# wamuumu/query-recommendation-system

Measured on AMD Instinct MI355X. Metric: MinHash signatures/sec through the whole hot path (signatures -> LSH candidates -> pair scoring -> top-K), higher is better.
Workload: dtype u16/int32 MinHash values, uint64 keys and pairs (integer); float64 cosine

## Files before the change

include/qrlsh.h:

```cpp
#ifndef QRLSH_H
#define QRLSH_H

#include <stddef.h>
#include <stdint.h>

#ifdef __cplusplus
extern "C" {
#endif

#define QRLSH_OK 0
#define QRLSH_EINVAL (-1)
#define QRLSH_EHIP (-2)
#define QRLSH_EUNSUPPORTED (-3)
#define QRLSH_EWORKSPACE (-4)

#define QRLSH_PERM_U16 0
#define QRLSH_PERM_I32 1

#define QRLSH_SIG_I32 0
#define QRLSH_SIG_U16 1

#define QRLSH_SORT_MIX 1u
#define QRLSH_SORT_IOTA 2u
#define QRLSH_SORT_FOLD 4u
// ... 65 lines not shown
                              void *stream);
int qrlsh_region_unique_fill(const uint64_t *tmp, int64_t n, int32_t group_bits, int64_t nids, const void *workspace,
                             uint64_t *out, void *stream);

size_t qrlsh_pair_regions_words(int64_t n, int64_t nids, int32_t group_bits, double words_per_query);
size_t qrlsh_pair_regions_tmp_words(int64_t n, int64_t nids, int32_t group_bits, double words_per_query);
int64_t qrlsh_pair_regions_cap(int64_t n, int64_t nids, int32_t group_bits, double words_per_query);
int64_t qrlsh_pair_regions_count(int64_t n, int64_t nids, int32_t group_bits, double words_per_query);
int qrlsh_pair_regions_scatter32(const uint64_t *words, int64_t n, int32_t group_bits, int32_t id_bits, int64_t nids,
                                 double words_per_query, uint64_t *tmp_regions, uint32_t *regions, uint32_t *counts,
                                 uint32_t *overflow_out, void *stream);
int qrlsh_region_unique_count_regions32(const uint32_t *regions, const uint32_t *counts, int64_t cap, int64_t n,
                                        int32_t group_bits, int32_t id_bits, int64_t nids, uint64_t *tmp, void *workspace,
                                        size_t workspace_bytes, const uint32_t *scatter_overflow, uint64_t *out3,
                                        void *stream);

int qrlsh_row_norms(const int32_t *sig, int64_t nq, int32_t P, int64_t *norm2_out, void *stream);
int qrlsh_verify_pairs(const void *sig, int32_t sig_dtype, int32_t P, int32_t b, const uint64_t *pairs,
                       int64_t n, uint8_t *flags_out, void *stream);
int qrlsh_score_pairs(const void *sig, int32_t sig_dtype, const int64_t *norm2, int32_t P,
                      const uint64_t *pairs, int64_t n, int32_t *milli_out, double *cos_out,
                      uint64_t *edge_out, int32_t id_bits, uint32_t *edge_dst_out, void *stream);

int qrlsh_topk_count(const uint64_t *sorted_edges, int64_t n_edges, int32_t K, int32_t id_bits,
                     void *workspace, size_t workspace_bytes, uint64_t *total_out, void *stream);
int qrlsh_topk_fill(const uint64_t *sorted_edges, const uint32_t *sorted_dst, int64_t n_edges, int32_t K,
                    int32_t id_bits, const void *workspace, int32_t *src_out, int32_t *dst_out,
                    int32_t *milli_out, void *stream);
int qrlsh_topk_fill_based(const uint64_t *sorted_edges, const uint32_t *sorted_dst, int64_t n_edges, int32_t K,
                          int32_t id_bits, int64_t src_base, const void *workspace, int32_t *src_out,
// ... 264 lines not shown
```

query-recommendation-system_amd/csrc/bucket.hip:

```cpp
#include "common.h"


__device__ static inline uint64_t rec_x(uint64_t word, int xbits) { return word & ((1ull << xbits) - 1ull); }
__device__ static inline uint64_t rec_word(uint64_t x, uint32_t id_hi, int xbits) {
  return rec_x(x, xbits) | (uint64_t)id_hi << xbits;
}
__device__ static inline uint32_t rec_id(uint64_t word, uint16_t tail, int xbits) {
  return (uint32_t)(word >> xbits) << 16 | tail;
}

struct PartPool {
  uint64_t *keys;
  uint16_t *vals;
  unsigned long long *cursor;
  uint32_t cap;
  uint4 *runs;
  unsigned long long *nruns;
  uint32_t runs_max;
  uint32_t *fill;
  uint32_t slot_base;
};

#ifndef QR_PS_IPT
#define QR_PS_IPT 16
// ... 790 lines not shown
QRLSH_EXPORT size_t qrlsh_bucket_part_words(int64_t nq, int32_t b, int32_t part_bits) {
  if (nq <= 0 || b <= 0) return 0;
  const size_t plain = (size_t)b * nq;
  const size_t regions = region_words(nq, b, part_bits) + pool_records(nq, b);
  return regions > plain ? regions : plain;
}
QRLSH_EXPORT size_t qrlsh_bucket_tmp_words(int64_t nq, int32_t b, int32_t part_bits) {
  if (nq <= 0 || b <= 0 || part_bits <= 8) return 0;
  const size_t plain = (size_t)b * nq;
  const int c1 = coarse_bits(part_bits);
  const int64_t slab = 1ll << slab_bits(part_bits);
  const size_t regions = (((size_t)b * n_slabs(nq, part_bits)) << c1) * coarse_region(nq < slab ? nq : slab, c1);
  return regions > plain ? regions : plain;
}

QRLSH_EXPORT int qrlsh_bucket_pairs_emit(const uint64_t *keys, uint64_t *part_keys, uint32_t *part_ids,
                                         uint64_t *tmp_keys, uint32_t *tmp_ids, int64_t nq, int32_t b, int32_t r,
                                         int32_t part_bits, void *workspace, size_t workspace_bytes,
                                         uint64_t *pairs_out, uint64_t capacity, uint64_t *total_overflow_out,
                                         void *stream) {
  return qrlsh_bucket_pairs_emit_chunked(keys, 0, 0, 0, part_keys, part_ids, tmp_keys, tmp_ids, nq, b, r, part_bits,
                                         workspace, workspace_bytes, pairs_out, capacity, total_overflow_out, stream);
}

QRLSH_EXPORT int qrlsh_bucket_pairs_emit_chunked(const uint64_t *keys, int64_t key_chunk, int64_t key_chunk_stride,
                                                 int64_t key_band_stride, uint64_t *part_keys, uint32_t *part_ids,
                                                 uint64_t *tmp_keys, uint32_t *tmp_ids, int64_t nq, int32_t b,
                                                 int32_t r, int32_t part_bits, void *workspace,
                                                 size_t workspace_bytes, uint64_t *pairs_out, uint64_t capacity,
                                                 uint64_t *total_overflow_out, void *stream) {
  QR_CHECK_ARG(key_chunk >= 0 && key_chunk_stride >= 0 && key_band_stride >= 0,
               "qrlsh_bucket_pairs_emit_chunked: bad key layout");
  hipStream_t st = static_cast<hipStream_t>(stream);
  const int rc = bucket_check("qrlsh_bucket_pairs_emit", keys, part_keys, part_ids, tmp_keys, tmp_ids, nq, b, r,
                              part_bits, workspace, workspace_bytes, total_overflow_out, st);
  if (rc != QRLSH_OK || nq == 0) return rc;
  QR_CHECK_ARG(pairs_out || capacity == 0, "qrlsh_bucket_pairs_emit: null output with capacity %llu",
               (unsigned long long)capacity);
  uint32_t *ovf = reinterpret_cast<uint32_t *>(total_overflow_out + 1);
  if (nq > (1ll << (16 + part_bits))) {
    if (hipMemsetAsync(ovf, 1, 1, st) != hipSuccess) {
      qrlsh_set_error("qrlsh_bucket_pairs_emit: hipMemsetAsync failed");
      return QRLSH_EHIP;
    }
    return QRLSH_OK;
  }
  const int nparts = 1 << part_bits;
  const BucketWs w = bucket_ws(workspace, nq, b, part_bits);
// ... 16 lines not shown
  pool.cap = (uint32_t)pool_records(nq, b);
  pool.runs = w.runs;
  pool.runs_max = POOL_RUNS;
  pool.fill = w.fill;
  pool.slot_base = 0;
  PartPool no_pool = pool;
  no_pool.keys = nullptr;
  no_pool.vals = nullptr;
  constexpr int MAX_GROUPS = EMIT_MAX_GROUPS;
  unsigned long long *nbig0 = w.nbig;
  uint64_t *biglist0 = w.biglist;
  const uint64_t slots = (uint64_t)b << T;
  const bool small_parts = two && small_form(nq, T);
  const int ntiles = (int)ceil_div64(nq, PS_TILE);
  const int64_t band_words = key_band_stride ? key_band_stride : nq;
  const int GROUPS = (int64_t)b * nq >= (64ll << 20) ? MAX_GROUPS : 1;
  const int per = (b + GROUPS - 1) / GROUPS;
  const int ngroups = (b + per - 1) / per;
  const uint64_t list_room = (slots - MAX_GROUPS) / (uint64_t)ngroups;
  const uint32_t big_max = (uint32_t)(list_room < FIN_BIG_LIST ? list_room : FIN_BIG_LIST);
  if (hipMemsetAsync(cur1, 0, (((size_t)b * nslabs) << c1) * sizeof(uint32_t), st) != hipSuccess ||
      (two && hipMemsetAsync(cur2, 0, ((size_t)b << T) * sizeof(uint32_t), st) != hipSuccess) ||
      hipMemsetAsync(w.fill, 0xFF, ((size_t)b << T) * sizeof(uint32_t), st) != hipSuccess ||
      hipMemsetAsync(w.poolctl, 0, 16, st) != hipSuccess ||
      hipMemsetAsync(nbig0, 0, MAX_GROUPS * sizeof(unsigned long long), st) != hipSuccess ||
      (ngroups > 1 && hipMemsetAsync(w.runs, 0, (size_t)POOL_RUNS * sizeof(uint4), st) != hipSuccess)) {
    qrlsh_set_error("qrlsh_bucket_pairs_emit: hipMemsetAsync failed");
    return QRLSH_EHIP;
  }
  hipStream_t aux = nullptr;
  int gi = 0;
  for (int g0 = 0; g0 < b; g0 += per, ++gi) {
    const int nb = (b - g0 < per) ? b - g0 : per;
    hipStream_t s = (aux && (gi & 1)) ? aux : st;
    uint64_t *biglist = biglist0 + (size_t)gi * big_max;
    unsigned long long *nbig = nbig0 + gi;
    uint64_t *k1 = two ? tmp_keys : part_keys;
    uint16_t *v1 = two ? tmp_tails : part_tails;
    pool.slot_base = (uint32_t)((size_t)g0 << T);
    BigDesc *desc = w.desc + (size_t)gi * FIN_BIG_LIST;
    const size_t in0 = ((size_t)g0 * nslabs) << c1;
    QR_PART_SCATTER(false, dim3(ntiles, nb), dim3(SORT_THREADS), 0, s, keys + (size_t)g0 * band_words,
                    (const uint16_t *)nullptr, k1 + in0 * cap1, v1 + in0 * cap1, nq, ntiles, 64 - c1, (1u << c1) - 1u,
                    cur1 + in0, cap1, ovf, qr_empty_key(r), (const uint32_t *)nullptr, 0u, key_chunk, key_chunk_stride,
                    key_band_stride, c1, nslabs, slab_shift, two ? no_pool : pool);
    if (two)
      QR_PART_SCATTER(true, dim3((unsigned)ceil_div64(cap1, PS_TILE), (nb * nslabs) << c1), dim3(SORT_THREADS), 0, s,
                      (const uint64_t *)tmp_keys + in0 * cap1, (const uint16_t *)tmp_tails + in0 * cap1,
                      part_keys + ((size_t)g0 << T) * cap2, part_tails + ((size_t)g0 << T) * cap2, (int64_t)0, 0, 64 - T,
                      lowmask, cur2 + ((size_t)g0 << T), cap2, ovf, qr_empty_key(r), (const uint32_t *)cur1 + in0, cap1,
                      (int64_t)0, (int64_t)0, (int64_t)0, c1, nslabs, slab_shift, pool);
    if (gi == 0 && b > per) aux = qr_aux_fork(st);
    const uint32_t slot0 = (uint32_t)((size_t)g0 << T);
    const uint64_t *gkeys = part_keys + (size_t)slot0 * cap2;
    const uint16_t *gids = part_tails + (size_t)slot0 * cap2;
    const uint32_t *gcounts = cur2 + slot0;
    if (small_parts && T >= 12)
      QR_LAUNCH("bucket_emit", bucket_finish_packed_kernel, dim3(nparts, nb), dim3(FIN_PK_THREADS), 0, s, gkeys, gids, nparts,
                64 - T, total_overflow_out, ovf, pairs_out, capacity, gcounts, cap2, biglist, nbig, big_max, slot0);
    else if (small_parts)
      QR_LAUNCH("bucket_emit", (bucket_finish_kernel<FIN_SMALL_THREADS, FIN_SMALL_CAP>), dim3(nparts, nb),
                dim3(FIN_SMALL_THREADS), 0, s, gkeys, gids, nparts, 64 - T, total_overflow_out, ovf, pairs_out, capacity, gcounts,
                cap2, biglist, nbig, big_max, slot0);
    else
      QR_LAUNCH("bucket_emit", (bucket_finish_kernel<>), dim3(nparts, nb), dim3(FIN_THREADS), 0, s, gkeys, gids, nparts, 64 - T,
                total_overflow_out, ovf, pairs_out, capacity, gcounts, cap2, biglist, nbig, big_max, slot0);
    QR_LAUNCH("bucket_emit_big", bucket_big_gather_kernel, dim3(64), dim3(256), 0, s, (const uint64_t *)biglist,
              (const unsigned long long *)nbig, big_max, desc, (const uint64_t *)part_keys, (const uint16_t *)part_tails,
              (const uint32_t *)cur2, cap2, pool, g_big_limit, ovf);
    QR_LAUNCH("bucket_emit_big", bucket_finish_big_kernel, dim3(FIN_BIG_GRID), dim3(FIN_THREADS), 0, s,
              (const uint64_t *)part_keys, (const uint16_t *)part_tails, (const uint64_t *)pool.keys,
              (const uint16_t *)pool.vals, 64 - T, (const BigDesc *)desc, (const unsigned long long *)nbig, big_max,
              total_overflow_out, pairs_out, capacity);
  }
  if (aux && qr_aux_join(st) != QRLSH_OK) return QRLSH_EHIP;
  QR_LAUNCH_CHECK("qrlsh_bucket_pairs_emit");
  return QRLSH_OK;
#undef QR_PART_SCATTER
}
```

query-recommendation-system_amd/csrc/dedup.hip:

```cpp
#include "common.h"
#include <type_traits>

struct RowSplit {
  int gbits, jbits;
  __device__ uint32_t row(uint64_t x) const { return (uint32_t)(x >> (32 + gbits)); }
  __device__ uint32_t val(uint64_t x) const {
    const uint32_t j = (uint32_t)x;
    return gbits ? ((uint32_t)(x >> 32) & ((1u << gbits) - 1u)) << jbits | j : j;
  }
  __device__ uint64_t word(uint64_t x0, uint32_t v) const {
    if (!gbits) return (x0 & 0xFFFFFFFF00000000ull) | v;
    const uint64_t i = ((x0 >> 32) & ~(uint64_t)((1u << gbits) - 1u)) | (v >> jbits);
    return i << 32 | (v & ((1u << jbits) - 1u));
  }
};

constexpr int RD_THREADS = 512;
constexpr int RD_C = 2048;
constexpr int RD_CAP = 1024;
constexpr int RD_IMG = RD_C + RD_CAP;
constexpr int RD_PER = RD_IMG / RD_THREADS;
constexpr uint32_t RD_EMPTY = 0xFFFFFFFFu;

__global__ __launch_bounds__(RD_THREADS) void row_unique_kernel(const uint64_t *__restrict__ in, int64_t n,
// ... 640 lines not shown
static_assert(PG_IPT_N2 % 4 == 0, "level 2 of the narrow form reads four entries per load");
static_assert(SORT_THREADS * (PG_IPT > PG_IPT_N1 ? (PG_IPT > PG_IPT_N2 ? PG_IPT : PG_IPT_N2) : (PG_IPT_N1 > PG_IPT_N2 ? PG_IPT_N1 : PG_IPT_N2)) < 0xFFFF,
              "a word's place in its tile is kept in 16 bits");
constexpr int PG_LDS_FIXED = RADIX * 9 + 16;
constexpr int pg_wgs(int ipt, int staged_bytes) {
  const int w = 160 * 1024 / (SORT_THREADS * ipt * staged_bytes + PG_LDS_FIXED);
  return w > 4 ? 4 : w < 1 ? 1 : w;
}
enum { PG_IN_WORDS = 0, PG_IN_TMP_NARROW = 2 };
enum { PG_OUT_VALUES = 1, PG_OUT_NARROW = 2 };
constexpr int pg_staged_bytes(int out) { return out == PG_OUT_VALUES ? 5 : 6; }
template <int IN, int OUT, int IPT>
__global__ __launch_bounds__(SORT_THREADS, pg_wgs(IPT, pg_staged_bytes(OUT))) void pair_group_scatter_kernel(
    const void *__restrict__ in_, const uint8_t *__restrict__ in_tails, void *__restrict__ out_, uint8_t *__restrict__ out_tails,
    int64_t n_in, int ntiles, int shift, uint32_t dmask, uint32_t *__restrict__ cursors, uint32_t cap,
    uint32_t *__restrict__ overflow, const uint32_t *__restrict__ in_counts, uint32_t in_cap, int gbits, int jbits, uint32_t bmask) {
  constexpr bool LEVEL2 = IN != PG_IN_WORDS;
  constexpr int TILE = SORT_THREADS * IPT;
  using D = typename std::conditional<OUT == PG_OUT_NARROW, uint16_t, uint8_t>::type;
  static_assert(IN == PG_IN_WORDS || IN == PG_IN_TMP_NARROW, "pair words or the tmp regions of a first level");
  static_assert(OUT == PG_OUT_NARROW ? IN == PG_IN_WORDS : OUT == PG_OUT_VALUES, "tmp regions are dealt into the final regions");
  __shared__ uint32_t cnt[RADIX];
  __shared__ uint32_t lsum[SORT_THREADS / WAVE];
  __shared__ uint32_t gdelta[RADIX];
  __shared__ uint8_t gok[RADIX];
  __shared__ __attribute__((aligned(16))) unsigned char stage[TILE * pg_staged_bytes(OUT)];
  uint32_t *const spay = reinterpret_cast<uint32_t *>(stage);
  D *const sdig = reinterpret_cast<D *>(stage + TILE * 4);
  const int tile = LEVEL2 ? (int)blockIdx.x : xcd_tile(blockIdx.x, ntiles), batch = blockIdx.y;
  const int lane = threadIdx.x & (WAVE - 1), w = threadIdx.x >> 6;
  const int64_t n = LEVEL2 ? (int64_t)min(in_counts[batch], in_cap) : n_in;
  const int64_t tbase = (int64_t)tile * TILE;
  if (tbase >= n) return;
  cnt[threadIdx.x] = 0;
  __syncthreads();
  const size_t boff = LEVEL2 ? (size_t)batch * in_cap : 0;
  const uint32_t nd = dmask + 1u;
  uint32_t pay[IPT];
  uint32_t dr[IPT];
  if constexpr (IN == PG_IN_TMP_NARROW) {
    const uint32_t *vals = static_cast<const uint32_t *>(in_) + boff;
    const uint8_t *tails = in_tails + boff;
    uint32_t tl[IPT / 4];
#pragma unroll
    for (int q = 0; q < IPT / 4; ++q) {
      const int64_t idx = tbase + ((int64_t)q * SORT_THREADS + threadIdx.x) * 4;
// ... 120 lines not shown
}
QRLSH_EXPORT size_t qrlsh_pair_regions_tmp_words(int64_t n, int64_t nids, int32_t group_bits, double words_per_query) {
  if (n <= 0 || nids <= 0 || group_bits < 0 || group_bits > 8) return 0;
  const PairRegions r = pair_regions(n, nids, group_bits, words_per_query);
  return r.ra ? (size_t)r.na * r.cap_a : 0;
}
QRLSH_EXPORT int64_t qrlsh_pair_regions_cap(int64_t n, int64_t nids, int32_t group_bits, double words_per_query) {
  if (n <= 0 || nids <= 0 || group_bits < 0 || group_bits > 8) return 0;
  return (int64_t)pair_regions(n, nids, group_bits, words_per_query).cap_b;
}
QRLSH_EXPORT int64_t qrlsh_pair_regions_count(int64_t n, int64_t nids, int32_t group_bits, double words_per_query) {
  if (n <= 0 || nids <= 0 || group_bits < 0 || group_bits > 8) return 0;
  return pair_regions(n, nids, group_bits, words_per_query).nregions;
}

QRLSH_EXPORT int qrlsh_pair_regions_scatter32(const uint64_t *words, int64_t n, int32_t group_bits, int32_t id_bits,
                                              int64_t nids, double words_per_query, uint64_t *tmp_regions, uint32_t *regions,
                                              uint32_t *counts, uint32_t *overflow_out, void *stream) {
  QR_CHECK_ARG(group_bits >= 0 && group_bits <= 8 && id_bits >= 1 && id_bits <= 31 && nids > 0 && nids <= (1ll << id_bits) &&
                   (group_bits + id_bits < 32 || (group_bits + id_bits == 32 && nids < (1ll << id_bits))),
               "qrlsh_pair_regions_scatter32: group_bits=%d / id_bits=%d / nids=%lld do not fit a 32-bit value", group_bits,
               id_bits, (long long)nids);
  QR_CHECK_ARG(n >= 0 && n < (1ll << 32) && counts && overflow_out, "qrlsh_pair_regions_scatter32: bad arguments");
  hipStream_t st = static_cast<hipStream_t>(stream);
  const PairRegions r = pair_regions(n > 0 ? n : 1, nids, group_bits, words_per_query);
  QR_CHECK_ARG(r.rbits <= 16 && r.na <= RADIX, "qrlsh_pair_regions_scatter32: %d region bits", r.rbits);
  QR_CHECK_ARG(pair_regions_fit_u32(r),
               "qrlsh_pair_regions_scatter32: regions reach 2^32 words (na * cap_a = %llu, 2^rb * cap_b = %llu; need both < 2^32)",
               (unsigned long long)r.na * r.cap_a, (unsigned long long)r.cap_b << r.rb);
  if (hipMemsetAsync(counts, 0, ((size_t)r.nregions + RADIX) * sizeof(uint32_t), st) != hipSuccess ||
      hipMemsetAsync(overflow_out, 0, sizeof(uint32_t), st) != hipSuccess) {
    qrlsh_set_error("qrlsh_pair_regions_scatter32: hipMemsetAsync failed");
    return QRLSH_EHIP;
  }
  if (n == 0) return QRLSH_OK;
  QR_CHECK_ARG(words && regions && (r.ra == 0 || tmp_regions), "qrlsh_pair_regions_scatter32: null pointer");
  const int sh = 32 + group_bits;
  const uint32_t *none = nullptr;
  if (r.ra == 0) {
    const int ntiles = (int)ceil_div64(n, SORT_THREADS * PG_IPT);
    QR_LAUNCH("pair_group", (pair_group_scatter_kernel<PG_IN_WORDS, PG_OUT_VALUES, PG_IPT>), dim3(ntiles, 1), dim3(SORT_THREADS), 0, st,
              (const void *)words, (const uint8_t *)nullptr, (void *)regions, (uint8_t *)nullptr, n, ntiles, sh,
              (1u << r.rb) - 1u, counts, r.cap_b, overflow_out, none, 0u, (int)group_bits, (int)id_bits, 0u);
  } else {
    QR_CHECK_ARG((reinterpret_cast<uintptr_t>(tmp_regions) & 15u) == 0, "qrlsh_pair_regions_scatter32: tmp_regions not 16-byte aligned");
    uint32_t *cur_a = counts + r.nregions;
    uint32_t *tvals = reinterpret_cast<uint32_t *>(tmp_regions);
    uint8_t *ttails = reinterpret_cast<uint8_t *>(tvals + (size_t)r.na * r.cap_a);
    const int ntiles = (int)ceil_div64(n, SORT_THREADS * PG_IPT_N1);
    QR_LAUNCH("pair_group", (pair_group_scatter_kernel<PG_IN_WORDS, PG_OUT_NARROW, PG_IPT_N1>), dim3(ntiles, 1), dim3(SORT_THREADS),
              0, st, (const void *)words, (const uint8_t *)nullptr, (void *)tvals, ttails, n, ntiles, sh + r.rb, (1u << r.ra) - 1u,
              cur_a, r.cap_a, overflow_out, none, 0u, (int)group_bits, (int)id_bits, (1u << r.rb) - 1u);
    QR_LAUNCH("pair_group", (pair_group_scatter_kernel<PG_IN_TMP_NARROW, PG_OUT_VALUES, PG_IPT_N2>),
              dim3((unsigned)ceil_div64(r.cap_a, SORT_THREADS * PG_IPT_N2), (unsigned)r.na), dim3(SORT_THREADS), 0, st,
              (const void *)tvals, (const uint8_t *)ttails, (void *)regions, (uint8_t *)nullptr, (int64_t)0, 0, 0, (1u << r.rb) - 1u,
              counts, r.cap_b, overflow_out, (const uint32_t *)cur_a, r.cap_a, 0, 0, 0u);
  }
  QR_LAUNCH_CHECK("qrlsh_pair_regions_scatter32");
  return QRLSH_OK;
}
```

query-recommendation-system_amd/qrlsh/_lib.py:

```python
import ctypes
import os

_HERE = os.path.dirname(os.path.abspath(__file__))
LIB_PATH = os.environ.get("QRLSH_LIB", os.path.join(_HERE, "libqrlsh.so"))

QRLSH_OK = 0
QRLSH_EINVAL = -1
QRLSH_EHIP = -2
QRLSH_EUNSUPPORTED = -3
QRLSH_EWORKSPACE = -4

PERM_U16 = 0
PERM_I32 = 1
SIG_I32 = 0
SIG_U16 = 1
SORT_MIX = 1
SORT_IOTA = 2
SORT_FOLD = 4
SORT_OWNER = 8
SORT_HOST = 16
SUM_PAIRWISE = 0
SUM_SEQUENTIAL = 1
RECOMMEND_MAX_K = 1024
INDEX_MAX_K = 256
# ... 29 lines not shown
    "qrlsh_bucket_part_words": (_sz, [_i64, _i32, _i32]),
    "qrlsh_set_big_part_limit": (_i64, [_i64]),
    "qrlsh_set_score_runs": (_i32, [_i32]),
    "qrlsh_bucket_tmp_words": (_sz, [_i64, _i32, _i32]),
    "qrlsh_bucket_pairs_emit": (ctypes.c_int, [_vp, _vp, _vp, _vp, _vp, _i64, _i32, _i32, _i32, _vp, _sz, _vp, _u64, _vp, _vp]),
    "qrlsh_compact_workspace_bytes": (_sz, [_i64]),
    "qrlsh_row_unique_workspace_bytes": (_sz, [_i64]),
    "qrlsh_row_unique_count": (ctypes.c_int, [_vp, _i64, _i32, _i32, _vp, _vp, _sz, _vp, _vp]),
    "qrlsh_row_unique_fill": (ctypes.c_int, [_vp, _i64, _vp, _vp, _vp]),
    "qrlsh_region_unique_workspace_bytes": (_sz, [_i64, _i32]),
    "qrlsh_region_unique_count": (ctypes.c_int, [_vp, _i64, _i32, _i32, _i64, _vp, _vp, _sz, _vp, _vp]),
    "qrlsh_region_unique_fill": (ctypes.c_int, [_vp, _i64, _i32, _i64, _vp, _vp, _vp]),
    "qrlsh_region_unique_count_regions32": (ctypes.c_int, [_vp, _vp, _i64, _i64, _i32, _i32, _i64, _vp, _vp, _sz, _vp, _vp,
                                                           _vp]),
    "qrlsh_pair_regions_scatter32": (ctypes.c_int, [_vp, _i64, _i32, _i32, _i64, ctypes.c_double, _vp, _vp, _vp, _vp, _vp]),
    "qrlsh_pair_regions_words": (_sz, [_i64, _i64, _i32, ctypes.c_double]),
    "qrlsh_pair_regions_tmp_words": (_sz, [_i64, _i64, _i32, ctypes.c_double]),
    "qrlsh_pair_regions_cap": (_i64, [_i64, _i64, _i32, ctypes.c_double]),
    "qrlsh_pair_regions_count": (_i64, [_i64, _i64, _i32, ctypes.c_double]),
    "qrlsh_unique_count": (ctypes.c_int, [_vp, _i64, _vp, _sz, _vp, _vp]),
    "qrlsh_unique_fill": (ctypes.c_int, [_vp, _i64, _vp, _vp, _vp]),
    "qrlsh_row_norms": (ctypes.c_int, [_vp, _i64, _i32, _vp, _vp]),
    "qrlsh_verify_pairs": (ctypes.c_int, [_vp, _i32, _i32, _i32, _vp, _i64, _vp, _vp]),
    "qrlsh_score_pairs": (ctypes.c_int, [_vp, _i32, _vp, _i32, _vp, _i64, _vp, _vp, _vp, _i32, _vp, _vp]),
    "qrlsh_remap_pairs": (ctypes.c_int, [_vp, _i64, _i64, _i64, _vp, _i64, _vp, _vp]),
    "qrlsh_pair_edges": (ctypes.c_int, [_vp, _vp, _i64, _i32, _vp, _vp, _vp, _vp, _vp]),
    "qrlsh_topk_count": (ctypes.c_int, [_vp, _i64, _i32, _i32, _vp, _sz, _vp, _vp]),
    "qrlsh_topk_fill": (ctypes.c_int, [_vp, _vp, _i64, _i32, _i32, _vp, _vp, _vp, _vp, _vp]),
    "qrlsh_topk_fill_based": (ctypes.c_int, [_vp, _vp, _i64, _i32, _i32, _i64, _vp, _vp, _vp, _vp, _vp]),
    "qrlsh_score_pairs_rev": (ctypes.c_int, [_vp, _i32, _vp, _i32, _vp, _i64, _vp, _vp, _i32, _vp, _vp]),
# ... 166 lines not shown
```

query-recommendation-system_amd/qrlsh/ops.py:

```python
import ctypes

import numpy as np
import torch

from . import _lib

_vp = ctypes.c_void_p


def _stream():
    return _vp(torch.cuda.current_stream().cuda_stream)


def _ptr(t):
    if t is None:
        return None
    return _vp(t.data_ptr())


def _need(t, dtype, name, ndim=None):
    if not isinstance(t, torch.Tensor) or not t.is_cuda:
        raise TypeError("%s must be a CUDA/HIP tensor" % name)
    if t.dtype != dtype:
        raise TypeError("%s must have dtype %s, got %s" % (name, dtype, t.dtype))
# ... 428 lines not shown
    while True:
        pairs = torch.empty((capacity,), dtype=torch.int64, device=dev)
        _lib.check(lib.qrlsh_bucket_pairs_emit_chunked(_ptr(keys), layout[0], layout[1], layout[2], _ptr(pk),
                                                       _ptr(pid), _ptr(tk), _ptr(tid), nq, b, r, T, _ptr(ws),
                                                       ws.numel(), _ptr(pairs), capacity, _ptr(tot), _stream()))
        n, overflow = tot.tolist()
        if overflow:
            return None
        _EMIT_HINT[shape] = n
        if n <= capacity:
            return pairs[:n]
        del pairs
        capacity = n


def emit_pairs_any(keys, r, stats=None):
    emitted = emit_pairs_fast(keys, r)
    if stats is not None:
        stats["bucket_path"] = "partition+lds" if emitted is not None else "general-sort"
        stats["part_bits"] = part_bits_for(keys.shape[1])
    if emitted is None:
        sk, sid = bucket_sort(keys)
        emitted = emit_pairs(sk, sid, r)
    return emitted


def verify_pairs(sig, b, pairs):
    lib = _lib.load()
    if not isinstance(sig, torch.Tensor) or sig.dtype not in (torch.int32, torch.int16):
        raise TypeError("sig must be an int32 or int16 (compact) tensor")
    _need(sig, sig.dtype, "sig", 2)
    _need(pairs, torch.int64, "pairs", 1)
    n = pairs.numel()
    flags = torch.empty((n,), dtype=torch.uint8, device=sig.device)
    code = _lib.SIG_U16 if sig.dtype == torch.int16 else _lib.SIG_I32
    _lib.check(lib.qrlsh_verify_pairs(_ptr(sig), code, sig.shape[1], b, _ptr(pairs), n, _ptr(flags), _stream()))
    return flags


def drop_unverified(sig, b, pairs, stats=None):
    if pairs.numel() == 0:
        return pairs
    flags = verify_pairs(sig, b, pairs)
    bad = int((flags == 0).sum().item())
    if stats is not None:
        stats["hash_collision_pairs_dropped"] = bad
    return pairs if bad == 0 else pairs[flags.bool()]


def candidate_pairs(keys, r, stats=None, sig=None):
    b, nq = keys.shape
    if r > 4 and sig is None:
        raise ValueError("band width r=%d > 4 needs the signatures for exact verification" % r)
    emitted = emit_pairs_any(keys, r, stats)
    if stats is not None:
        stats["emitted_pairs"] = int(emitted.numel())
    if emitted.numel() == 0:
        return emitted
    pairs = unique_pairs(emitted, nq, stats)
    if r > 4:
        pairs = drop_unverified(sig, b, pairs, stats)
    return pairs


def wide_ids(id_bits):
    return 2 * id_bits + 11 > 64


def score_pairs(sig, norm2, pairs, want_cos=False, edge_id_bits=None, wide=None):
    lib = _lib.load()
    if not isinstance(sig, torch.Tensor) or sig.dtype not in (torch.int32, torch.int16):
        raise TypeError("sig must be an int32 or int16 (compact) tensor")
    _need(sig, sig.dtype, "sig", 2)
    if norm2 is not None:
# ... 668 lines not shown
```

Baseline: 670.0 million.

## Emit pairs into per-band-group segments and scatter them straight into dedup regions

Adds a segmented emit path. Each band group writes its pairs into its own preallocated segment with a device-side counter. The region scatter kernel then reads each segment's count from device memory, so the emit capacity no longer has to be read back on the host and the emitted buffer no longer has to be trimmed before dedup. Candidate generation uses this path when a size hint from an earlier call exists. It avoids host synchronisation and extra passes between emit and dedup. In exchange it carries more complex fallback logic and over-allocates segment capacity from per-shape hints.

```diff
diff --git a/include/qrlsh.h b/include/qrlsh.h
--- a/include/qrlsh.h
+++ b/include/qrlsh.h
@@ -103,6 +103,18 @@
                                         int32_t group_bits, int32_t id_bits, int64_t nids, uint64_t *tmp, void *workspace,
                                         size_t workspace_bytes, const uint32_t *scatter_overflow, uint64_t *out3,
                                         void *stream);
+
+int qrlsh_bucket_pairs_emit_segments(const uint64_t *keys, uint64_t *part_keys, uint32_t *part_ids, uint64_t *tmp_keys,
+                                     uint32_t *tmp_ids, int64_t nq, int32_t b, int32_t r, int32_t part_bits,
+                                     void *workspace, size_t workspace_bytes, uint64_t *pairs_out,
+                                     const uint64_t *seg_caps, uint64_t *seg_counts, uint64_t *total_overflow_out,
+                                     void *stream);
+int qrlsh_pair_regions_scatter32_segments(const uint64_t *words, const uint64_t *seg_caps, const uint64_t *seg_counts,
+                                          int32_t nseg, int64_t n_hint, int32_t group_bits, int32_t id_bits, int64_t nids,
+                                          double words_per_query, uint64_t *tmp_regions, uint32_t *regions,
+                                          uint32_t *counts, uint32_t *overflow_out, void *stream);
+int32_t qrlsh_bucket_group_bands(int64_t nq, int32_t b);
+int qrlsh_set_force_band_groups(int on);
 
 int qrlsh_row_norms(const int32_t *sig, int64_t nq, int32_t P, int64_t *norm2_out, void *stream);
 int qrlsh_verify_pairs(const void *sig, int32_t sig_dtype, int32_t P, int32_t b, const uint64_t *pairs,
diff --git a/query-recommendation-system_amd/csrc/bucket.hip b/query-recommendation-system_amd/csrc/bucket.hip
--- a/query-recommendation-system_amd/csrc/bucket.hip
+++ b/query-recommendation-system_amd/csrc/bucket.hip
@@ -828,6 +828,15 @@
   return regions > plain ? regions : plain;
 }
 
+struct QrEmitSegments {
+  const uint64_t *seg_caps;
+  uint64_t *seg_counts;
+};
+static int qr_bucket_emit(const uint64_t *keys, int64_t key_chunk, int64_t key_chunk_stride, int64_t key_band_stride,
+                          uint64_t *part_keys, uint32_t *part_ids, uint64_t *tmp_keys, uint32_t *tmp_ids, int64_t nq, int32_t b,
+                          int32_t r, int32_t part_bits, void *workspace, size_t workspace_bytes, uint64_t *pairs_out,
+                          uint64_t capacity, uint64_t *total_overflow_out, const QrEmitSegments *segs, hipStream_t st);
+
 QRLSH_EXPORT int qrlsh_bucket_pairs_emit(const uint64_t *keys, uint64_t *part_keys, uint32_t *part_ids,
                                          uint64_t *tmp_keys, uint32_t *tmp_ids, int64_t nq, int32_t b, int32_t r,
                                          int32_t part_bits, void *workspace, size_t workspace_bytes,
@@ -843,9 +852,47 @@
                                                  int32_t r, int32_t part_bits, void *workspace,
                                                  size_t workspace_bytes, uint64_t *pairs_out, uint64_t capacity,
                                                  uint64_t *total_overflow_out, void *stream) {
+  return qr_bucket_emit(keys, key_chunk, key_chunk_stride, key_band_stride, part_keys, part_ids, tmp_keys, tmp_ids, nq, b, r,
+                        part_bits, workspace, workspace_bytes, pairs_out, capacity, total_overflow_out, nullptr,
+                        static_cast<hipStream_t>(stream));
+}
+
+QRLSH_EXPORT int qrlsh_bucket_pairs_emit_segments(const uint64_t *keys, uint64_t *part_keys, uint32_t *part_ids,
+                                                  uint64_t *tmp_keys, uint32_t *tmp_ids, int64_t nq, int32_t b, int32_t r,
+                                                  int32_t part_bits, void *workspace, size_t workspace_bytes,
+                                                  uint64_t *pairs_out, const uint64_t *seg_caps, uint64_t *seg_counts,
+                                                  uint64_t *total_overflow_out, void *stream) {
+  const QrEmitSegments segs{seg_caps, seg_counts};
+  return qr_bucket_emit(keys, 0, 0, 0, part_keys, part_ids, tmp_keys, tmp_ids, nq, b, r, part_bits, workspace, workspace_bytes,
+                        pairs_out, 0, total_overflow_out, &segs, static_cast<hipStream_t>(stream));
+}
+
+static int g_force_groups = 0;
+QRLSH_EXPORT int qrlsh_set_force_band_groups(int on) {
+  const int old = g_force_groups;
+  g_force_groups = on != 0;
+  return old;
+}
+static int emit_groups(int64_t nq, int32_t b) {
+  return (g_force_groups || (int64_t)b * nq >= (64ll << 20)) ? EMIT_MAX_GROUPS : 1;
+}
+QRLSH_EXPORT int32_t qrlsh_bucket_group_bands(int64_t nq, int32_t b) {
+  if (b <= 0) return 0;
+  const int groups = emit_groups(nq, b);
+  return (b + groups - 1) / groups;
+}
+
+static int qr_bucket_emit(const uint64_t *keys, int64_t key_chunk, int64_t key_chunk_stride, int64_t key_band_stride,
+                          uint64_t *part_keys, uint32_t *part_ids, uint64_t *tmp_keys, uint32_t *tmp_ids, int64_t nq, int32_t b,
+                          int32_t r, int32_t part_bits, void *workspace, size_t workspace_bytes, uint64_t *pairs_out,
+                          uint64_t capacity, uint64_t *total_overflow_out, const QrEmitSegments *segs, hipStream_t st) {
   QR_CHECK_ARG(key_chunk >= 0 && key_chunk_stride >= 0 && key_band_stride >= 0,
                "qrlsh_bucket_pairs_emit_chunked: bad key layout");
-  hipStream_t st = static_cast<hipStream_t>(stream);
+  QR_CHECK_ARG(!segs || (segs->seg_caps && segs->seg_counts), "qrlsh_bucket_pairs_emit: segments without capacities or cursors");
+  if (segs && hipMemsetAsync(segs->seg_counts, 0, EMIT_MAX_GROUPS * sizeof(uint64_t), st) != hipSuccess) {
+    qrlsh_set_error("qrlsh_bucket_pairs_emit: hipMemsetAsync failed");
+    return QRLSH_EHIP;
+  }
   const int rc = bucket_check("qrlsh_bucket_pairs_emit", keys, part_keys, part_ids, tmp_keys, tmp_ids, nq, b, r,
                               part_bits, workspace, workspace_bytes, total_overflow_out, st);
   if (rc != QRLSH_OK || nq == 0) return rc;
@@ -892,7 +939,7 @@
   const bool small_parts = two && small_form(nq, T);
   const int ntiles = (int)ceil_div64(nq, PS_TILE);
   const int64_t band_words = key_band_stride ? key_band_stride : nq;
-  const int GROUPS = (int64_t)b * nq >= (64ll << 20) ? MAX_GROUPS : 1;
+  const int GROUPS = emit_groups(nq, b);
   const int per = (b + GROUPS - 1) / GROUPS;
   const int ngroups = (b + per - 1) / per;
   const uint64_t list_room = (slots - MAX_GROUPS) / (uint64_t)ngroups;
@@ -908,9 +955,13 @@
   }
   hipStream_t aux = nullptr;
   int gi = 0;
+  uint64_t seg_off = 0;
   for (int g0 = 0; g0 < b; g0 += per, ++gi) {
     const int nb = (b - g0 < per) ? b - g0 : per;
     hipStream_t s = (aux && (gi & 1)) ? aux : st;
+    uint64_t *const gcur = segs ? segs->seg_counts + gi : total_overflow_out;
+    uint64_t *const gout = segs ? pairs_out + seg_off : pairs_out;
+    const uint64_t gcap = segs ? segs->seg_caps[gi] : capacity;
     uint64_t *biglist = biglist0 + (size_t)gi * big_max;
     unsigned long long *nbig = nbig0 + gi;
     uint64_t *k1 = two ? tmp_keys : part_keys;
@@ -935,21 +986,22 @@
     const uint32_t *gcounts = cur2 + slot0;
     if (small_parts && T >= 12)
       QR_LAUNCH("bucket_emit", bucket_finish_packed_kernel, dim3(nparts, nb), dim3(FIN_PK_THREADS), 0, s, gkeys, gids, nparts,
-                64 - T, total_overflow_out, ovf, pairs_out, capacity, gcounts, cap2, biglist, nbig, big_max, slot0);
+                64 - T, gcur, ovf, gout, gcap, gcounts, cap2, biglist, nbig, big_max, slot0);
     else if (small_parts)
       QR_LAUNCH("bucket_emit", (bucket_finish_kernel<FIN_SMALL_THREADS, FIN_SMALL_CAP>), dim3(nparts, nb),
-                dim3(FIN_SMALL_THREADS), 0, s, gkeys, gids, nparts, 64 - T, total_overflow_out, ovf, pairs_out, capacity, gcounts,
+                dim3(FIN_SMALL_THREADS), 0, s, gkeys, gids, nparts, 64 - T, gcur, ovf, gout, gcap, gcounts,
                 cap2, biglist, nbig, big_max, slot0);
     else
       QR_LAUNCH("bucket_emit", (bucket_finish_kernel<>), dim3(nparts, nb), dim3(FIN_THREADS), 0, s, gkeys, gids, nparts, 64 - T,
-                total_overflow_out, ovf, pairs_out, capacity, gcounts, cap2, biglist, nbig, big_max, slot0);
+                gcur, ovf, gout, gcap, gcounts, cap2, biglist, nbig, big_max, slot0);
     QR_LAUNCH("bucket_emit_big", bucket_big_gather_kernel, dim3(64), dim3(256), 0, s, (const uint64_t *)biglist,
               (const unsigned long long *)nbig, big_max, desc, (const uint64_t *)part_keys, (const uint16_t *)part_tails,
               (const uint32_t *)cur2, cap2, pool, g_big_limit, ovf);
     QR_LAUNCH("bucket_emit_big", bucket_finish_big_kernel, dim3(FIN_BIG_GRID), dim3(FIN_THREADS), 0, s,
               (const uint64_t *)part_keys, (const uint16_t *)part_tails, (const uint64_t *)pool.keys,
               (const uint16_t *)pool.vals, 64 - T, (const BigDesc *)desc, (const unsigned long long *)nbig, big_max,
-              total_overflow_out, pairs_out, capacity);
+              gcur, gout, gcap);
+    if (segs) seg_off += gcap;
   }
   if (aux && qr_aux_join(st) != QRLSH_OK) return QRLSH_EHIP;
   QR_LAUNCH_CHECK("qrlsh_bucket_pairs_emit");
diff --git a/query-recommendation-system_amd/csrc/dedup.hip b/query-recommendation-system_amd/csrc/dedup.hip
--- a/query-recommendation-system_amd/csrc/dedup.hip
+++ b/query-recommendation-system_amd/csrc/dedup.hip
@@ -678,7 +678,8 @@
 __global__ __launch_bounds__(SORT_THREADS, pg_wgs(IPT, pg_staged_bytes(OUT))) void pair_group_scatter_kernel(
     const void *__restrict__ in_, const uint8_t *__restrict__ in_tails, void *__restrict__ out_, uint8_t *__restrict__ out_tails,
     int64_t n_in, int ntiles, int shift, uint32_t dmask, uint32_t *__restrict__ cursors, uint32_t cap,
-    uint32_t *__restrict__ overflow, const uint32_t *__restrict__ in_counts, uint32_t in_cap, int gbits, int jbits, uint32_t bmask) {
+    uint32_t *__restrict__ overflow, const uint32_t *__restrict__ in_counts, uint32_t in_cap, int gbits, int jbits, uint32_t bmask,
+    const unsigned long long *__restrict__ n_dev) {
   constexpr bool LEVEL2 = IN != PG_IN_WORDS;
   constexpr int TILE = SORT_THREADS * IPT;
   using D = typename std::conditional<OUT == PG_OUT_NARROW, uint16_t, uint8_t>::type;
@@ -693,7 +694,16 @@
   D *const sdig = reinterpret_cast<D *>(stage + TILE * 4);
   const int tile = LEVEL2 ? (int)blockIdx.x : xcd_tile(blockIdx.x, ntiles), batch = blockIdx.y;
   const int lane = threadIdx.x & (WAVE - 1), w = threadIdx.x >> 6;
-  const int64_t n = LEVEL2 ? (int64_t)min(in_counts[batch], in_cap) : n_in;
+  int64_t n = LEVEL2 ? (int64_t)min(in_counts[batch], in_cap) : n_in;
+  if constexpr (!LEVEL2)
+    if (n_dev) {
+      const unsigned long long c = *n_dev;
+      if (c > (unsigned long long)n_in) {
+        if (blockIdx.x == 0 && threadIdx.x == 0) atomicOr(overflow, 1u);
+        return;
+      }
+      n = (int64_t)c;
+    }
   const int64_t tbase = (int64_t)tile * TILE;
   if (tbase >= n) return;
   cnt[threadIdx.x] = 0;
@@ -844,48 +854,98 @@
   return pair_regions(n, nids, group_bits, words_per_query).nregions;
 }
 
-QRLSH_EXPORT int qrlsh_pair_regions_scatter32(const uint64_t *words, int64_t n, int32_t group_bits, int32_t id_bits,
-                                              int64_t nids, double words_per_query, uint64_t *tmp_regions, uint32_t *regions,
-                                              uint32_t *counts, uint32_t *overflow_out, void *stream) {
-  QR_CHECK_ARG(group_bits >= 0 && group_bits <= 8 && id_bits >= 1 && id_bits <= 31 && nids > 0 && nids <= (1ll << id_bits) &&
-                   (group_bits + id_bits < 32 || (group_bits + id_bits == 32 && nids < (1ll << id_bits))),
-               "qrlsh_pair_regions_scatter32: group_bits=%d / id_bits=%d / nids=%lld do not fit a 32-bit value", group_bits,
-               id_bits, (long long)nids);
-  QR_CHECK_ARG(n >= 0 && n < (1ll << 32) && counts && overflow_out, "qrlsh_pair_regions_scatter32: bad arguments");
-  hipStream_t st = static_cast<hipStream_t>(stream);
-  const PairRegions r = pair_regions(n > 0 ? n : 1, nids, group_bits, words_per_query);
-  QR_CHECK_ARG(r.rbits <= 16 && r.na <= RADIX, "qrlsh_pair_regions_scatter32: %d region bits", r.rbits);
-  QR_CHECK_ARG(pair_regions_fit_u32(r),
-               "qrlsh_pair_regions_scatter32: regions reach 2^32 words (na * cap_a = %llu, 2^rb * cap_b = %llu; need both < 2^32)",
-               (unsigned long long)r.na * r.cap_a, (unsigned long long)r.cap_b << r.rb);
-  if (hipMemsetAsync(counts, 0, ((size_t)r.nregions + RADIX) * sizeof(uint32_t), st) != hipSuccess ||
-      hipMemsetAsync(overflow_out, 0, sizeof(uint32_t), st) != hipSuccess) {
-    qrlsh_set_error("qrlsh_pair_regions_scatter32: hipMemsetAsync failed");
-    return QRLSH_EHIP;
-  }
-  if (n == 0) return QRLSH_OK;
-  QR_CHECK_ARG(words && regions && (r.ra == 0 || tmp_regions), "qrlsh_pair_regions_scatter32: null pointer");
+static int pg_level1(const char *name, const PairRegions &r, const uint64_t *words, int64_t n, const unsigned long long *n_dev,
+                     int32_t group_bits, int32_t id_bits, uint64_t *tmp_regions, uint32_t *regions, uint32_t *counts,
+                     uint32_t *overflow_out, hipStream_t st) {
   const int sh = 32 + group_bits;
   const uint32_t *none = nullptr;
   if (r.ra == 0) {
     const int ntiles = (int)ceil_div64(n, SORT_THREADS * PG_IPT);
     QR_LAUNCH("pair_group", (pair_group_scatter_kernel<PG_IN_WORDS, PG_OUT_VALUES, PG_IPT>), dim3(ntiles, 1), dim3(SORT_THREADS), 0, st,
               (const void *)words, (const uint8_t *)nullptr, (void *)regions, (uint8_t *)nullptr, n, ntiles, sh,
-              (1u << r.rb) - 1u, counts, r.cap_b, overflow_out, none, 0u, (int)group_bits, (int)id_bits, 0u);
+              (1u << r.rb) - 1u, counts, r.cap_b, overflow_out, none, 0u, (int)group_bits, (int)id_bits, 0u, n_dev);
   } else {
-    QR_CHECK_ARG((reinterpret_cast<uintptr_t>(tmp_regions) & 15u) == 0, "qrlsh_pair_regions_scatter32: tmp_regions not 16-byte aligned");
     uint32_t *cur_a = counts + r.nregions;
     uint32_t *tvals = reinterpret_cast<uint32_t *>(tmp_regions);
     uint8_t *ttails = reinterpret_cast<uint8_t *>(tvals + (size_t)r.na * r.cap_a);
     const int ntiles = (int)ceil_div64(n, SORT_THREADS * PG_IPT_N1);
     QR_LAUNCH("pair_group", (pair_group_scatter_kernel<PG_IN_WORDS, PG_OUT_NARROW, PG_IPT_N1>), dim3(ntiles, 1), dim3(SORT_THREADS),
               0, st, (const void *)words, (const uint8_t *)nullptr, (void *)tvals, ttails, n, ntiles, sh + r.rb, (1u << r.ra) - 1u,
-              cur_a, r.cap_a, overflow_out, none, 0u, (int)group_bits, (int)id_bits, (1u << r.rb) - 1u);
-    QR_LAUNCH("pair_group", (pair_group_scatter_kernel<PG_IN_TMP_NARROW, PG_OUT_VALUES, PG_IPT_N2>),
-              dim3((unsigned)ceil_div64(r.cap_a, SORT_THREADS * PG_IPT_N2), (unsigned)r.na), dim3(SORT_THREADS), 0, st,
-              (const void *)tvals, (const uint8_t *)ttails, (void *)regions, (uint8_t *)nullptr, (int64_t)0, 0, 0, (1u << r.rb) - 1u,
-              counts, r.cap_b, overflow_out, (const uint32_t *)cur_a, r.cap_a, 0, 0, 0u);
-  }
-  QR_LAUNCH_CHECK("qrlsh_pair_regions_scatter32");
+              cur_a, r.cap_a, overflow_out, none, 0u, (int)group_bits, (int)id_bits, (1u << r.rb) - 1u, n_dev);
+  }
+  QR_LAUNCH_CHECK(name);
   return QRLSH_OK;
 }
+
+static int pg_level2(const char *name, const PairRegions &r, uint64_t *tmp_regions, uint32_t *regions, uint32_t *counts,
+                     uint32_t *overflow_out, hipStream_t st) {
+  if (r.ra == 0) return QRLSH_OK;
+  uint32_t *cur_a = counts + r.nregions;
+  uint32_t *tvals = reinterpret_cast<uint32_t *>(tmp_regions);
+  uint8_t *ttails = reinterpret_cast<uint8_t *>(tvals + (size_t)r.na * r.cap_a);
+  QR_LAUNCH("pair_group", (pair_group_scatter_kernel<PG_IN_TMP_NARROW, PG_OUT_VALUES, PG_IPT_N2>),
+            dim3((unsigned)ceil_div64(r.cap_a, SORT_THREADS * PG_IPT_N2), (unsigned)r.na), dim3(SORT_THREADS), 0, st,
+            (const void *)tvals, (const uint8_t *)ttails, (void *)regions, (uint8_t *)nullptr, (int64_t)0, 0, 0, (1u << r.rb) - 1u,
+            counts, r.cap_b, overflow_out, (const uint32_t *)cur_a, r.cap_a, 0, 0, 0u, (const unsigned long long *)nullptr);
+  QR_LAUNCH_CHECK(name);
+  return QRLSH_OK;
+}
+
+static int pg_begin(const char *name, int64_t n, int32_t group_bits, int32_t id_bits, int64_t nids, double words_per_query,
+                    uint32_t *counts, uint32_t *overflow_out, hipStream_t st, PairRegions *out) {
+  QR_CHECK_ARG(group_bits >= 0 && group_bits <= 8 && id_bits >= 1 && id_bits <= 31 && nids > 0 && nids <= (1ll << id_bits) &&
+                   (group_bits + id_bits < 32 || (group_bits + id_bits == 32 && nids < (1ll << id_bits))),
+               "%s: group_bits=%d / id_bits=%d / nids=%lld do not fit a 32-bit value", name, group_bits, id_bits, (long long)nids);
+  QR_CHECK_ARG(n >= 0 && n < (1ll << 32) && counts && overflow_out, "%s: bad arguments", name);
+  const PairRegions r = pair_regions(n > 0 ? n : 1, nids, group_bits, words_per_query);
+  QR_CHECK_ARG(r.rbits <= 16 && r.na <= RADIX, "%s: %d region bits", name, r.rbits);
+  QR_CHECK_ARG(pair_regions_fit_u32(r), "%s: regions reach 2^32 words (na * cap_a = %llu, 2^rb * cap_b = %llu; need both < 2^32)",
+               name, (unsigned long long)r.na * r.cap_a, (unsigned long long)r.cap_b << r.rb);
+  if (hipMemsetAsync(counts, 0, ((size_t)r.nregions + RADIX) * sizeof(uint32_t), st) != hipSuccess ||
+      hipMemsetAsync(overflow_out, 0, sizeof(uint32_t), st) != hipSuccess) {
+    qrlsh_set_error("%s: hipMemsetAsync failed", name);
+    return QRLSH_EHIP;
+  }
+  *out = r;
+  return QRLSH_OK;
+}
+static int pg_pointers(const char *name, const PairRegions &r, const void *words, const uint64_t *tmp_regions, const uint32_t *regions) {
+  QR_CHECK_ARG(words && regions && (r.ra == 0 || tmp_regions), "%s: null pointer", name);
+  QR_CHECK_ARG(r.ra == 0 || (reinterpret_cast<uintptr_t>(tmp_regions) & 15u) == 0, "%s: tmp_regions not 16-byte aligned", name);
+  return QRLSH_OK;
+}
+
+QRLSH_EXPORT int qrlsh_pair_regions_scatter32(const uint64_t *words, int64_t n, int32_t group_bits, int32_t id_bits,
+                                              int64_t nids, double words_per_query, uint64_t *tmp_regions, uint32_t *regions,
+                                              uint32_t *counts, uint32_t *overflow_out, void *stream) {
+  const char *name = "qrlsh_pair_regions_scatter32";
+  hipStream_t st = static_cast<hipStream_t>(stream);
+  PairRegions r;
+  int rc = pg_begin(name, n, group_bits, id_bits, nids, words_per_query, counts, overflow_out, st, &r);
+  if (rc != QRLSH_OK || n == 0) return rc;
+  if ((rc = pg_pointers(name, r, words, tmp_regions, regions)) != QRLSH_OK) return rc;
+  rc = pg_level1(name, r, words, n, nullptr, group_bits, id_bits, tmp_regions, regions, counts, overflow_out, st);
+  return rc != QRLSH_OK ? rc : pg_level2(name, r, tmp_regions, regions, counts, overflow_out, st);
+}
+
+QRLSH_EXPORT int qrlsh_pair_regions_scatter32_segments(const uint64_t *words, const uint64_t *seg_caps,
+                                                       const uint64_t *seg_counts, int32_t nseg, int64_t n_hint,
+                                                       int32_t group_bits, int32_t id_bits, int64_t nids,
+                                                       double words_per_query, uint64_t *tmp_regions, uint32_t *regions,
+                                                       uint32_t *counts, uint32_t *overflow_out, void *stream) {
+  const char *name = "qrlsh_pair_regions_scatter32_segments";
+  hipStream_t st = static_cast<hipStream_t>(stream);
+  QR_CHECK_ARG(seg_caps && seg_counts && nseg >= 1 && nseg <= 2 && n_hint > 0, "%s: bad arguments", name);
+  PairRegions r;
+  int rc = pg_begin(name, n_hint, group_bits, id_bits, nids, words_per_query, counts, overflow_out, st, &r);
+  if (rc != QRLSH_OK || (rc = pg_pointers(name, r, words, tmp_regions, regions)) != QRLSH_OK) return rc;
+  uint64_t off = 0;
+  for (int k = 0; k < nseg; off += seg_caps[k], ++k) {
+    if (seg_caps[k] == 0) continue;
+    QR_CHECK_ARG(seg_caps[k] < (1ull << 32), "%s: segment of %llu words", name, (unsigned long long)seg_caps[k]);
+    rc = pg_level1(name, r, words + off, (int64_t)seg_caps[k], reinterpret_cast<const unsigned long long *>(seg_counts + k),
+                   group_bits, id_bits, tmp_regions, regions, counts, overflow_out, st);
+    if (rc != QRLSH_OK) return rc;
+  }
+  return pg_level2(name, r, tmp_regions, regions, counts, overflow_out, st);
+}
diff --git a/query-recommendation-system_amd/qrlsh/_lib.py b/query-recommendation-system_amd/qrlsh/_lib.py
--- a/query-recommendation-system_amd/qrlsh/_lib.py
+++ b/query-recommendation-system_amd/qrlsh/_lib.py
@@ -67,6 +67,12 @@
     "qrlsh_region_unique_count_regions32": (ctypes.c_int, [_vp, _vp, _i64, _i64, _i32, _i32, _i64, _vp, _vp, _sz, _vp, _vp,
                                                            _vp]),
     "qrlsh_pair_regions_scatter32": (ctypes.c_int, [_vp, _i64, _i32, _i32, _i64, ctypes.c_double, _vp, _vp, _vp, _vp, _vp]),
+    "qrlsh_bucket_pairs_emit_segments": (ctypes.c_int, [_vp, _vp, _vp, _vp, _vp, _i64, _i32, _i32, _i32, _vp, _sz, _vp, _vp, _vp, _vp,
+                                                        _vp]),
+    "qrlsh_pair_regions_scatter32_segments": (ctypes.c_int, [_vp, _vp, _vp, _i32, _i64, _i32, _i32, _i64, ctypes.c_double, _vp, _vp,
+                                                             _vp, _vp, _vp]),
+    "qrlsh_bucket_group_bands": (_i32, [_i64, _i32]),
+    "qrlsh_set_force_band_groups": (ctypes.c_int, [ctypes.c_int]),
     "qrlsh_pair_regions_words": (_sz, [_i64, _i64, _i32, ctypes.c_double]),
     "qrlsh_pair_regions_tmp_words": (_sz, [_i64, _i64, _i32, ctypes.c_double]),
     "qrlsh_pair_regions_cap": (_i64, [_i64, _i64, _i32, ctypes.c_double]),
diff --git a/query-recommendation-system_amd/qrlsh/ops.py b/query-recommendation-system_amd/qrlsh/ops.py
--- a/query-recommendation-system_amd/qrlsh/ops.py
+++ b/query-recommendation-system_amd/qrlsh/ops.py
@@ -466,11 +466,11 @@
         capacity = n
 
 
-def emit_pairs_any(keys, r, stats=None):
-    emitted = emit_pairs_fast(keys, r)
+def emit_pairs_any(keys, r, stats=None, part_bits=None):
+    emitted = emit_pairs_fast(keys, r, part_bits=part_bits)
     if stats is not None:
         stats["bucket_path"] = "partition+lds" if emitted is not None else "general-sort"
-        stats["part_bits"] = part_bits_for(keys.shape[1])
+        stats["part_bits"] = part_bits if part_bits is not None else part_bits_for(keys.shape[1])
     if emitted is None:
         sk, sid = bucket_sort(keys)
         emitted = emit_pairs(sk, sid, r)
@@ -500,16 +500,122 @@
     return pairs if bad == 0 else pairs[flags.bool()]
 
 
-def candidate_pairs(keys, r, stats=None, sig=None):
+_SEG_HINT = {}
+_GROUP_REFUSED = set()
+
+
+def emit_segment_caps(nq, b, r, hint):
+    lib = _lib.load()
+    per = lib.qrlsh_bucket_group_bands(nq, b)
+    bands = [min(per, b - g0) for g0 in range(0, b, per)]
+    last = _SEG_HINT.get((nq, b, r))
+    if last is None or len(last) != len(bands):
+        last = [-(-hint * nb // b) for nb in bands]
+    return [c * 5 // 4 + 1024 for c in last]
+
+
+def emit_group_pairs(keys, r, hint, stats=None, part_bits=None, seg_caps=None):
+    lib = _lib.load()
+    _need(keys, torch.int64, "keys", 2)
+    b, nq = keys.shape
+    dev = keys.device
+    T = part_bits if part_bits is not None else part_bits_for(nq)
+    ib = id_bits_for(nq)
+    hint = int(hint)
+    if hint <= 0 or nq == 0 or nq > 6144 * (1 << T) or hint >= (1 << 32):
+        return None
+    wpq = hint / nq
+    g = region_group_bits(ib, nq, wpq)
+    if g is None or g < REGION_MIN_GROUP_BITS or not region_values_fit(g, ib, nq):
+        return None
+    words = lib.qrlsh_pair_regions_words(hint, nq, g, wpq)
+    twords = lib.qrlsh_pair_regions_tmp_words(hint, nq, g, wpq)
+    if words == 0 or words * 12 + twords * 8 > REGION_SCATTER_MAX_BYTES:
+        return None
+    shape = (nq, b, r)
+    if seg_caps is None:
+        seg_caps = emit_segment_caps(nq, b, r, hint)
+    per = lib.qrlsh_bucket_group_bands(nq, b)
+    ngroups = -(-b // per)
+    if len(seg_caps) != ngroups or max(seg_caps) >= (1 << 32):
+        return None
+    cap = lib.qrlsh_pair_regions_cap(hint, nq, g, wpq)
+    nreg = lib.qrlsh_pair_regions_count(hint, nq, g, wpq)
+    pwords = lib.qrlsh_bucket_part_words(nq, b, T)
+    bwords = lib.qrlsh_bucket_tmp_words(nq, b, T) if T > 8 else 0
+    res = torch.zeros(8, dtype=torch.int64, device=dev)
+    seg_counts, tot = res.data_ptr() + 40, res.data_ptr() + 24
+    caps_host = (ctypes.c_uint64 * len(seg_caps))(*seg_caps)
+    caps_ptr = ctypes.cast(caps_host, ctypes.c_void_p)
+    counts = torch.empty((nreg + 256,), dtype=torch.int32, device=dev)
+    ovf = torch.empty((1,), dtype=torch.int32, device=dev)
+    try:
+        pk = torch.empty((pwords,), dtype=torch.int64, device=dev)
+        pid = torch.empty((pwords,), dtype=torch.int32, device=dev)
+        tk = torch.empty((bwords,), dtype=torch.int64, device=dev) if T > 8 else None
+        tid = torch.empty((bwords,), dtype=torch.int32, device=dev) if T > 8 else None
+        bws = _ws(lib.qrlsh_bucket_workspace_bytes(nq, b, T), dev)
+        pairs = torch.empty((sum(seg_caps),), dtype=torch.int64, device=dev)
+        _lib.check(lib.qrlsh_bucket_pairs_emit_segments(_ptr(keys), _ptr(pk), _ptr(pid), _ptr(tk), _ptr(tid), nq, b, r, T,
+                                                        _ptr(bws), bws.numel(), _ptr(pairs), caps_ptr, seg_counts, tot,
+                                                        _stream()))
+        del pk, pid, tk, tid, bws
+        regions = torch.empty((words,), dtype=torch.int32, device=dev)
+        tmpr = torch.empty((twords,), dtype=torch.int64, device=dev) if twords else None
+        _lib.check(lib.qrlsh_pair_regions_scatter32_segments(_ptr(pairs), caps_ptr, seg_counts, ngroups, hint, int(g),
+                                                             int(ib), int(nq), wpq, _ptr(tmpr), _ptr(regions),
+                                                             _ptr(counts), _ptr(ovf), _stream()))
+        tmp =torch.empty((words,), dtype=torch.int64, device=dev)
+    except torch.cuda.OutOfMemoryError:
+        pk = pid = tk = tid = bws = pairs = regions = tmpr = tmp = None
+        torch.cuda.synchronize()
+        torch.cuda.empty_cache()
+        return None
+    del tmpr
+    ws = _ws(lib.qrlsh_region_unique_workspace_bytes(nq, g), dev)
+    _lib.check(lib.qrlsh_region_unique_count_regions32(_ptr(regions), _ptr(counts), cap, hint, int(g), int(ib), int(nq),
+                                                       _ptr(tmp), _ptr(ws), ws.numel(), _ptr(ovf), _ptr(res), _stream()))
+    total, distinct, capped, _, part_ovf, c0, c1, _ = res.tolist()
+    segs = [c0, c1][:ngroups]
+    if not part_ovf:
+        _EMIT_HINT[shape] = sum(segs)
+        _SEG_HINT[shape] = segs
+    if not part_ovf and any(c > room for c, room in zip(segs, seg_caps)):
+        return None
+    if part_ovf or capped or distinct:
+        _GROUP_REFUSED.add(shape)
+        return None
+    if stats is not None:
+        stats["bucket_path"] = "partition+lds"
+        stats["part_bits"] = T
+        stats["emitted_pairs"] = sum(segs)
+        stats["dedup_path"] = "regions-in-lds (scattered)"
+        stats["group_bits"] = g
+    del regions, pairs
+    out = torch.empty((total,), dtype=torch.int64, device=dev)
+    _lib.check(lib.qrlsh_region_unique_fill(_ptr(tmp), hint, int(g), int(nq), _ptr(ws), _ptr(out), _stream()))
+    return out
+
+
+def candidate_pairs(keys, r, stats=None, sig=None, part_bits=None):
     b, nq = keys.shape
     if r > 4 and sig is None:
         raise ValueError("band width r=%d > 4 needs the signatures for exact verification" % r)
-    emitted = emit_pairs_any(keys, r, stats)
-    if stats is not None:
-        stats["emitted_pairs"] = int(emitted.numel())
+    shape = (nq, b, r)
+    hint = _EMIT_HINT.get(shape, 0) if r <= 4 else 0
+    if hint > 0 and shape not in _GROUP_REFUSED:
+        pairs = emit_group_pairs(keys, r, hint, stats, part_bits=part_bits)
+        if pairs is not None:
+            return pairs
+    if stats is None:
+        stats = {}
+    emitted = emit_pairs_any(keys, r, stats, part_bits=part_bits)
+    stats["emitted_pairs"] = int(emitted.numel())
     if emitted.numel() == 0:
         return emitted
     pairs = unique_pairs(emitted, nq, stats)
+    if stats["bucket_path"] == "partition+lds" and stats["dedup_path"] == "regions-in-lds (scattered)":
+        _GROUP_REFUSED.discard(shape)
     if r > 4:
         pairs = drop_unverified(sig, b, pairs, stats)
     return pairs
```

Result: slower. 655.6 million (-2.2%).
